# HuttleyLab/DiverseSeq

Hardware: AMD Instinct MI355X
Metric: sequences scored/sec (delta-JSD, k=6) (higher is better)
Workload: dtype f64 (results and every set update in f64; reject/accept decisions tiered: f32 and f32-log scores decide rows farther from the threshold than their proven error bands, f64 the rest)

## Files before the change

### diverseseq_amd/csrc/persist.hip

```cpp
#include "select_dev.h"

#include <algorithm>
#include <type_traits>
#include <cstddef>
#include <cstdlib>
#include <cstring>

namespace {

constexpr int P_THREADS = 512;
constexpr int P_J = 8;
constexpr int P_CH = 16;
constexpr uint32_t P_MAXN = 512;
constexpr uint32_t P_MAXN_BIG = 256;
constexpr uint32_t P_MAXN_MAX = 896;
constexpr uint32_t p_maxn(bool cached, bool maxm = false) { return cached ? (maxm ? P_MAXN_MAX : P_MAXN) : P_MAXN_BIG; }
constexpr uint32_t P_SMALLN = 16;
constexpr uint32_t P_SMALL_ROWS = 13;
constexpr uint32_t p_maxjobs(bool cached, bool maxm = false) { return p_maxn(cached, maxm) + 1; }
constexpr size_t p_acc_bytes(uint32_t maxn) { return size_t(8) * (maxn + 1) * 2 * sizeof(unsigned long long); }
__device__ __forceinline__ unsigned long long p_acc_word(double v) {
    return ((unsigned long long)__double2ll_rn(v * 0x1p50) << 6) + 1ull;
}
__device__ __forceinline__ double p_acc_value(unsigned long long w) { return double((long long)w >> 6) * 0x1p-50; }
// ... 2790 lines not shown
                        rec = __hip_atomic_load(&sync->wrec[epoch & 1u][q], RLX_AGENT);
                    if (p_word_listed(rec) != (l2 ? 1u : 0u)) wrong = true;
                    if (l2) {
                        unsigned long long ent = __hip_atomic_load(&sync->soft[epoch & 1u][q][0], RLX_AGENT);
                        for (uint32_t spins = 0; !p_word_is(ent, epoch) && spins < (1u << 20); spins++)
                            ent = __hip_atomic_load(&sync->soft[epoch & 1u][q][0], RLX_AGENT);
                        if (p_word_pos(ent, epoch) != uint64_t(epoch) * 4096u + 4001u + q) wrong = true;
                    }
                }
            }
            if (__ballot(wrong) != 0ull && lane == 0) fails++;
        }
        for (uint32_t z = (h >> 20) & 7u; z > 0; z--) __builtin_amdgcn_s_sleep(2);
        if (b < HO_MEMBERS * HO_K && tid < 8) {
            const double v = double((h >> 4) & 0xFFFFu) * (1.0 / 65536.0), v2 = double(h & 0xFFu) * (1.0 / 4096.0);
            p_acc_add(acc_all + (uint64_t(tid) * (HO_MEMBERS + 1) + b / HO_K) * 2, v, v2);
        }
        bool acc_ok = true, acc_wrong = false;
        if (tid < HO_MEMBERS) {
            const unsigned long long d0 = p_acc_complete(acc + uint64_t(tid) * 2, s_prev + tid * 2, HO_K, acc_ok);
            const unsigned long long d1 = p_acc_complete(acc + uint64_t(tid) * 2 + 1, s_prev + tid * 2 + 1, HO_K, acc_ok);
            unsigned long long e0 = 0ull, e1 = 0ull;
            for (uint32_t q = 0; q < HO_K; q++) {
                const uint32_t h2 = ho_hash(epoch, tid * HO_K + q);
                e0 += p_acc_word(double((h2 >> 4) & 0xFFFFu) * (1.0 / 65536.0));
                e1 += p_acc_word(double(h2 & 0xFFu) * (1.0 / 4096.0));
            }
            acc_wrong = !acc_ok || d0 != e0 || d1 != e1;
        }
        if (__syncthreads_or(acc_wrong ? 1 : 0) && tid == 0) fails++;
        if (mirror && epoch + 1 < rounds) {
            if (tid == 0) __hip_atomic_store(&sync->wrec[(epoch + 1) & 1u][b], p_word(epoch + 1, SEL_NONE, false), RLX_AGENT);
            early_rec = epoch + 1;
            for (uint32_t z = (h >> 16) & 15u; z > 0; z--) __builtin_amdgcn_s_sleep(16);
        }
    }
    if (tid == 0 && fails) atomicAdd(bad, fails);
    if (tid == 0 && __hip_atomic_load(&sync->timeout, RLX_AGENT)) atomicAdd(bad, 1ull << 32);
}

}

template <typename T>
static const void *persist_fn(const dvs_select *s) {
    const bool cached = s->dev.B <= uint64_t(P_J) * P_THREADS;
    if (s->params.mode == DVS_MODE_MAX) return reinterpret_cast<const void *>(persist_nmost_kernel<T, true, true>);
    if constexpr (std::is_same_v<T, uint16_t>) {
        if (s->persist_small) return reinterpret_cast<const void *>(persist_nmost_kernel<T, true, false, true>);
    }
    return cached ? reinterpret_cast<const void *>(persist_nmost_kernel<T, true>)
                  : reinterpret_cast<const void *>(persist_nmost_kernel<T, false>);
}

static int persist_prepare(dvs_ctx *ctx, dvs_select *s, uint32_t head_stop, hipStream_t on) {
    std::vector<unsigned char> &image = head_stop ? s->h_psync_head : s->h_psync;
    image.assign(sizeof(PSync), 0);
    PSync &init = *reinterpret_cast<PSync *>(image.data());
    init.stop_at = head_stop;
    init.seeded = s->persist_seeded ? 1u : 0u;
    init.seed_list = static_cast<const unsigned long long *>(s->d_seed_list);
    for (int g = 0; g < 8; g++) init.rel[g].hint = ~0ull;
    init.wg_thresh = s->params.window ? 0u : 4u;
    init.wg_scale = 1.5f;
    if (ctx->knobs.persist_wg_rounds >= 0) init.wg_thresh = uint32_t(ctx->knobs.persist_wg_rounds);
    init.no_coarse = (ctx->knobs.persist_no_coarse ? 1u : 0u) | (ctx->knobs.persist_no_events ? 2u : 0u) |
                     0u;
    init.small_rows = s->persist_small ? s->persist_small_rows : 0u;
    init.lds_bytes = uint32_t(s->persist_lds);
    init.wmax = uint32_t(std::min<uint64_t>(s->npos, 0xFFFFFFFFull));
    DVS_HIP(ctx, hipMemcpyAsync(head_stop ? s->psync_head : s->psync, &init, sizeof init, hipMemcpyHostToDevice, on));
    DVS_HIP(ctx, hipMemsetAsync(head_stop ? s->ppart_head : s->ppart, 0, p_acc_bytes(s->persist_maxn), on));
    return DVS_OK;
}

template <typename T>
static int persist_launch(dvs_ctx *ctx, dvs_select *s, const T *mat, uint32_t grid, uint32_t head_stop,
                          hipStream_t on) {
    const SelDev &d = s->dev;
    if (head_stop ? !s->head_prepared : !s->persist_prepared) {
        int prc = persist_prepare(ctx, s, head_stop, on);
        if (prc) return prc;
    }
    if (head_stop) s->head_prepared = false;
    else s->persist_prepared = false;
    s->persist_seeded = false;
    hipEvent_t e0 = nullptr, e1 = nullptr;
    if (s->time_scan) {
        if (s->ev_used + 2 > s->ev_pool.size()) {
            hipEvent_t a = dvs_event_get(ctx), b = dvs_event_get(ctx);
            s->ev_pool.push_back(a);
            s->ev_pool.push_back(b);
        }
        e0 = s->ev_pool[s->ev_used];
        e1 = s->ev_pool[s->ev_used + 1];
        s->ev_used += 2;
        (void)hipEventRecord(e0, on);
    }
    const void *fn = persist_fn<T>(s);
    SelDev d_arg = d;
    const T *mat_arg = mat;
    PSync *sync_arg = static_cast<PSync *>(head_stop ? s->psync_head : s->psync);
    unsigned long long *part_arg = static_cast<unsigned long long *>(head_stop ? s->ppart_head : s->ppart);
    uint32_t g_arg = grid;
    void *args[] = {&d_arg, &mat_arg, &sync_arg, &part_arg, &g_arg};
    hipError_t le = hipLaunchKernel(fn, dim3(grid), dim3(P_THREADS), args, s->persist_lds, on);
    if (s->time_scan) (void)hipEventRecord(e1, on);
    if (le != hipSuccess) {
        (void)hipGetLastError();
        return DVS_ERR_UNSUPPORTED;
    }
    DVS_HIP(ctx, hipGetLastError());
    return DVS_OK;
}

int dvs_persist_setup(dvs_ctx *ctx, dvs_select *s) {
    const uint64_t B = s->dev.B;
    s->persist = false;
    if (ctx->knobs.no_persist || ctx->persist_timeouts >= 3) return DVS_OK;
    if (ctx->knobs.cu_mask_set) return DVS_OK;
    const bool maxm = s->params.mode == DVS_MODE_MAX;
    if ((s->params.mode != DVS_MODE_NMOST && !maxm) || !s->h_order.empty() || !s->h_labels.empty()) return DVS_OK;
    if (s->npos >= P_POS_NONE) return DVS_OK;
    s->persist_grid = uint32_t(std::min(ctx->n_cu, int(P_MAXG)));
    const bool cached = B <= uint64_t(P_J) * P_THREADS;
    if (maxm && !cached) return DVS_OK;
// ... 31 lines not shown
        auto hit = ctx->persist_fits.find(key);
        if (hit == ctx->persist_fits.end()) {
            int per_cu = 0;
            const bool fits = hipOccupancyMaxActiveBlocksPerMultiprocessor(&per_cu, fn, P_THREADS, lds) == hipSuccess && per_cu >= 1;
            if (!fits) (void)hipGetLastError();
            hit = ctx->persist_fits.emplace(key, fits).first;
        }
        if (!hit->second) return DVS_OK;
    }
    rc = dvs_dev_alloc(ctx, &s->psync, sizeof(PSync), "persistent sync block");
    if (!rc) rc = dvs_dev_alloc(ctx, &s->ppart, p_acc_bytes(s->persist_maxn) + (maxm ? 2 * p_batch_bytes() : 0),
                                "leave-one-out accumulators");
    if (rc) return rc;
    s->persist = true;
    return DVS_OK;
}

size_t dvs_persist_dbg_offset(void) { return offsetof(PSync, dbg2); }
#ifdef DVS_PERSIST_STAMPS
size_t dvs_persist_trace_offset(void) { return offsetof(PSync, trace); }
#else
size_t dvs_persist_trace_offset(void) { return 0; }
#endif
#if defined(DVS_PERSIST_STAMPS) && defined(DVS_PROBE)
int dvs_persist_probe_id(void) { return DVS_PROBE; }
#else
int dvs_persist_probe_id(void) { return 0; }
#endif

int dvs_persist_launch(dvs_ctx *ctx, dvs_select *s) {
    return dvs_mat_dispatch(s->mat, [&](auto *mp) { return persist_launch(ctx, s, mp, s->persist_grid, 0u, ctx->stream); });
}

static int persist_head_blocks(dvs_ctx *ctx, dvs_select *s) {
    if (s->psync_head) return DVS_OK;
    int rc = dvs_dev_alloc(ctx, &s->psync_head, sizeof(PSync), "head phase sync block");
    if (!rc) rc = dvs_dev_alloc(ctx, &s->ppart_head, p_acc_bytes(s->persist_maxn), "head phase accumulators");
    return rc;
}

int dvs_persist_launch_head(dvs_ctx *ctx, dvs_select *s, uint32_t grid, uint32_t stop_at, hipStream_t on) {
    int rc = persist_head_blocks(ctx, s);
    if (rc) return rc;
    return dvs_mat_dispatch(s->mat, [&](auto *mp) { return persist_launch(ctx, s, mp, grid, stop_at, on); });
}

int dvs_persist_prepare_head(dvs_ctx *ctx, dvs_select *s, uint32_t stop_at, hipStream_t on) {
    int rc = persist_head_blocks(ctx, s);
    if (!rc) rc = persist_prepare(ctx, s, stop_at, on);
    if (!rc) s->head_prepared = true;
    return rc;
}

int dvs_persist_prepare_main(dvs_ctx *ctx, dvs_select *s) {
    int rc = persist_prepare(ctx, s, 0u, ctx->stream);
    if (!rc) s->persist_prepared = true;
    return rc;
}

extern "C" int dvs_selftest_handover(dvs_ctx *ctx, uint32_t rounds, uint64_t *failures) {
    if (!ctx || !failures || !rounds) return dvs_set_error(ctx, DVS_ERR_VALUE, "bad argument");
    if (rounds >= P_EPOCH_MAX) return dvs_set_error(ctx, DVS_ERR_VALUE, "at most %u rounds", P_EPOCH_MAX - 1);
    DVS_HIP(ctx, hipSetDevice(ctx->device));
    const uint32_t G = uint32_t(std::min(ctx->n_cu, int(P_MAXG)));
    if (G < HO_MEMBERS * HO_K + 2 || ctx->knobs.cu_mask_set)
        return dvs_set_error(ctx, DVS_ERR_UNSUPPORTED, "the self-test wants %u co-resident workgroups", HO_MEMBERS * HO_K + 2);
    void *d_sync = nullptr, *d_acc = nullptr, *d_bad = nullptr;
    int rc = dvs_dev_alloc(ctx, &d_sync, sizeof(PSync), "self-test sync block");
    if (!rc) rc = dvs_dev_alloc(ctx, &d_acc, p_acc_bytes(HO_MEMBERS), "self-test accumulators");
    if (!rc) rc = dvs_dev_alloc(ctx, &d_bad, 8, "self-test counter");
    if (!rc) {
        std::vector<unsigned char> image(sizeof(PSync), 0);
        PSync &init = *reinterpret_cast<PSync *>(image.data());
        for (int g = 0; g < 8; g++) init.rel[g].hint = ~0ull;
        hipError_t e = hipMemcpyAsync(d_sync, image.data(), sizeof(PSync), hipMemcpyHostToDevice, ctx->stream);
        if (e == hipSuccess) e = hipMemsetAsync(d_acc, 0, p_acc_bytes(HO_MEMBERS), ctx->stream);
        if (e == hipSuccess) e = hipMemsetAsync(d_bad, 0, 8, ctx->stream);
        if (e == hipSuccess) e = hipStreamSynchronize(ctx->stream);
        if (e == hipSuccess) {
            hipLaunchKernelGGL(handover_selftest_kernel, dim3(G), dim3(P_THREADS), 0, ctx->stream, static_cast<PSync *>(d_sync),
                               static_cast<unsigned long long *>(d_acc), G, rounds, static_cast<unsigned long long *>(d_bad));
            e = hipGetLastError();
        }
        unsigned long long bad = 0;
        if (e == hipSuccess) e = hipMemcpyAsync(&bad, d_bad, 8, hipMemcpyDeviceToHost, ctx->stream);
        if (e == hipSuccess) e = hipStreamSynchronize(ctx->stream);
        if (e != hipSuccess) rc = dvs_hip_fail(ctx, e, "hand-over self-test");
        *failures = bad;
    }
    dvs_dev_free(ctx, d_sync);
    dvs_dev_free(ctx, d_acc);
    dvs_dev_free(ctx, d_bad);
    return rc;
}
```

### diverseseq_amd/csrc/select.h

```cpp
#pragma once

#include "dvs_internal.h"

#define SEL_NONE 0xFFFFFFFFFFFFFFFFull
#define SEL_SEEDS_AT 512

enum : uint32_t { SEL_RUN = 0, SEL_DONE = 1, SEL_ARBITER = 2, SEL_ERROR = 3,
                  SEL_NEED_SETUP = 4 };
enum : uint32_t { ARB_RESOLVE = 1, ARB_FINALIZE = 2 };
enum : uint32_t { FORCE_NONE = 0, FORCE_ACCEPT = 1, FORCE_REJECT = 2, FORCE_COMMIT = 3, FORCE_ROLLBACK = 4 };

struct SelCtl {
    unsigned long long cursor;
    unsigned long long npos;
    unsigned long long event_pos;
    unsigned long long arb_pos;
    unsigned long long rows_scored, rows_rechecked;
    unsigned long long rows_coarse_passed;
    unsigned long long rows_before_launch;
    uint32_t window, window_min, window_max;
    uint32_t status, arb_stage, forced, forced_lowest;
    uint32_t size, lowest, mode, max_size, stat;
    uint32_t ev_kind;
    uint32_t ev_n;
// ... 18 lines not shown
    SelCtl *ctl = nullptr;
    uint64_t B = 0;
    uint32_t nlabels = 0;
    const uint32_t *order = nullptr;
    const uint32_t *labels = nullptr;
    const uint32_t *totals = nullptr;
    const double *rowH = nullptr;
    double *S = nullptr;
    double *Stmp = nullptr;
    double *base = nullptr;
    double *cand = nullptr;
    double *M = nullptr;
    double *mH = nullptr;
    double *mDelta = nullptr;
    double *dtmp = nullptr;
    double *dsum = nullptr;
    uint32_t *mLabel = nullptr;
    unsigned long long *mPos = nullptr;
    uint32_t *ord = nullptr;
    uint8_t *inset = nullptr;
    uint32_t *wg_rows = nullptr;
    unsigned long long *evlog_pos = nullptr;
    uint32_t *evlog_kind = nullptr;
    const double *gather_all = nullptr;
    uint32_t gather_world = 0;
    double *rowlog = nullptr;
    uint32_t rowlog_cap = 0;
};

struct dvs_select {
    dvs_ctx *ctx = nullptr;
    dvs_select_params params{};
    const dvs_matrix *mat = nullptr;
    int mat_kind = 0;
    uint64_t npos = 0;
    uint32_t cap = 0;
    SelDev dev;
    SelCtl *h_ctl = nullptr;
    SelCtl ctl0{};
    std::vector<uint32_t> h_order, h_labels;
    std::vector<uint32_t> h_out_labels;
    std::vector<uint64_t> seed_positions;
    uint32_t scan_grid = 0, loo_grid = 0;
    size_t scan_lds = 0;
    bool base_in_lds = true;
    bool scan_hot = false;
    bool persist = false;
    bool persist_fell_back = false;
    uint32_t persist_grid = 0, persist_maxn = 0, persist_maxjobs = 0;
    bool persist_small = false;
    uint32_t persist_small_rows = 0;
    size_t persist_lds = 0;
    void *psync = nullptr;
    std::vector<unsigned char> h_psync;
    std::vector<unsigned char> h_psync_head;
    void *ppart = nullptr;
    double *d_mbres = nullptr;
    uint32_t mb_jw = 0;
    uint32_t mb_launched = 0;
    void *psync_head = nullptr, *ppart_head = nullptr;
    bool persist_seeded = false;
    bool seeded_start = false;
    bool head_prepared = false;
    bool persist_prepared = false;
    bool used_side_streams = false;
    hipEvent_t ev_side_done = nullptr;
    void *d_seed_list = nullptr;
    bool seed_list_in_ctl = false;
    bool inset_clean = false;
    hipStream_t setup_side = nullptr;
    bool head_phase = false;
    int batch = 16;
    bool time_scan = false;
    std::vector<hipEvent_t> ev_pool;
    size_t ev_used = 0;
    double scan_ms = 0.0;
    double scan_ms_last = 0.0;
    uint64_t scan_launches = 0;
    uint32_t n_arbitrated = 0;
    double arbiter_ms = 0.0;
    bool fast_step = false;
    bool fs_need_scan = false;
    unsigned long long *h_fshist = nullptr;
    unsigned long long fs_launches = 0;
    unsigned long long fs_peek_floor = 0;
    double *fs_slot = nullptr;
    double *fs_packed = nullptr;
    double *d_jobres = nullptr;
    void *d_fsync = nullptr;
    uint32_t fs_K = 1, fs_jobs = 0, fs_grid = 0;
    size_t fs_lds = 0;
    std::vector<double> h_rowlog;
    uint64_t rowlog_have = 0;
    uint32_t steps_since_poll = 0;
    void *arbiter = nullptr;
};

int dvs_select_arbitrate(dvs_ctx *ctx, dvs_select *s);
void dvs_select_arbiter_free(dvs_select *s);

int dvs_persist_setup(dvs_ctx *ctx, dvs_select *s);
int dvs_persist_launch(dvs_ctx *ctx, dvs_select *s);
int dvs_persist_launch_head(dvs_ctx *ctx, dvs_select *s, uint32_t grid, uint32_t stop_at, hipStream_t on);
int dvs_persist_prepare_main(dvs_ctx *ctx, dvs_select *s);
int dvs_persist_prepare_head(dvs_ctx *ctx, dvs_select *s, uint32_t stop_at, hipStream_t on);
size_t dvs_persist_dbg_offset(void);
size_t dvs_persist_trace_offset(void);
int dvs_persist_probe_id(void);
```

### diverseseq_amd/csrc/select.hip

```cpp
#include "dvs_internal.h"
#include "select.h"
#include "select_dev.h"

#include <algorithm>
#include <chrono>
#include <type_traits>
#include <cmath>
#include <cstring>
#include <cstdlib>

namespace {

constexpr int SCAN_THREADS = 512;
constexpr int WIDE_THREADS = 1024;
constexpr int LOO_THREADS = 256;

template <typename T>
__device__ __forceinline__ void scan_rows_hot(SelCtl *ctl, const T *__restrict__ mat,
                                              const uint32_t *__restrict__ totals,
                                              const double *__restrict__ rowH, const double *bvec,
                                              uint64_t B, const ScanState &st, uint64_t first,
                                              uint64_t stride, uint32_t lane, uint32_t &nread,
                                              uint32_t &nprecise) {
    for (uint64_t r = first; r < st.nrows; r += stride) {
// ... 1693 lines not shown
}

__global__ __launch_bounds__(LOO_THREADS) void gather_members_kernel(SelDev d, double *__restrict__ rows,
                                                                    double *__restrict__ meta) {
    const uint32_t r = blockIdx.x, n = d.ctl->size;
    double *out = rows + uint64_t(r) * d.B;
    if (r >= n) {
        for (uint64_t i = threadIdx.x; i < d.B; i += LOO_THREADS) out[i] = 0.0;
        if (threadIdx.x == 0) meta[2 * r] = meta[2 * r + 1] = 0.0;
        return;
    }
    const uint32_t slot = d.ord[r];
    const double *src = d.M + uint64_t(slot) * d.B;
    for (uint64_t i = threadIdx.x; i < d.B; i += LOO_THREADS) out[i] = src[i];
    if (threadIdx.x == 0) {
        meta[2 * r] = double(d.mPos[slot]);
        meta[2 * r + 1] = 1.0;
    }
}

template <typename T>
__global__ __launch_bounds__(LOO_THREADS) void pack_event_kernel(SelDev d, const T *__restrict__ mat,
                                                                double *__restrict__ slot) {
    pack_event_body<T>(d, mat, slot);
}

}

static void sel_free(dvs_select *s) {
    if (!s) return;
#ifdef DVS_FS_TRACE
    if (s->d_jobres && getenv("DVS_FS_DEBUG")) {
        std::vector<unsigned long long> t(8 * 1024);
        (void)hipDeviceSynchronize();
        if (hipMemcpy(t.data(), reinterpret_cast<char *>(s->d_jobres) + size_t(2048) * 8 * 8, t.size() * 8, hipMemcpyDeviceToHost) == hipSuccess) {
            unsigned long long t0 = ~0ull;
            for (uint32_t b = 0; b < s->fs_grid; b++) if (t[b * 8]) t0 = std::min(t0, t[b * 8]);
            auto us = [&](unsigned long long x) { return x ? (double(x) - double(t0)) / 100.0 : -1.0; };
            double mx[8] = {0}, mn[8]; for (int k = 0; k < 8; k++) mn[k] = 1e9;
            for (uint32_t b = 1; b < s->fs_grid; b++) for (int k = 0; k < 7; k++) if (t[b * 8 + k]) { mx[k] = std::max(mx[k], us(t[b * 8 + k])); mn[k] = std::min(mn[k], us(t[b * 8 + k])); }
            fprintf(stderr, "[fs trace] scanning workgroups (us, min/max): start %.1f/%.1f decided %.1f/%.1f base+arrived %.1f/%.1f scan end %.1f/%.1f\n", mn[0], mx[0], mn[1], mx[1], mn[2], mx[2], mn[6], mx[6]);
            std::vector<double> e, r1, c1, sc; double posted = -1; unsigned long long nr = 0, nrmax = 0;
            for (uint32_t b = 1; b < s->fs_grid; b++) { if (t[b * 8 + 6]) e.push_back(us(t[b * 8 + 6])); if (t[b * 8 + 3]) r1.push_back(us(t[b * 8 + 3])); if (t[b * 8 + 4]) c1.push_back(us(t[b * 8 + 4]));
                if (t[b * 8 + 5]) sc.push_back(us(t[b * 8 + 5])); nr += t[b * 8 + 7]; nrmax = std::max(nrmax, t[b * 8 + 7]); }
            std::sort(e.begin(), e.end()); std::sort(r1.begin(), r1.end()); std::sort(c1.begin(), c1.end()); std::sort(sc.begin(), sc.end());
            auto pc = [&](std::vector<double> &v, double q) { return v.empty() ? -1.0 : v[size_t(q * (v.size() - 1))]; };
            fprintf(stderr, "[fs trace] wave 0s: scan loop entered p10/50/90/max %.1f %.1f %.1f %.1f; first row's data there %.1f %.1f %.1f %.1f; its score %.1f %.1f %.1f %.1f; scan end %.1f %.1f %.1f %.1f; first post (wave 0s only) %.1f; rows read sum %llu max %llu\n",
                    pc(sc, .1), pc(sc, .5), pc(sc, .9), pc(sc, 1), pc(r1, .1), pc(r1, .5), pc(r1, .9), pc(r1, 1), pc(c1, .1), pc(c1, .5), pc(c1, .9), pc(c1, 1), pc(e, .1), pc(e, .5), pc(e, .9), pc(e, 1), posted, nr, nrmax);
            const uint32_t L = 0;
            fprintf(stderr, "[fs trace] state writer: start %.1f decided %.1f loaded %.1f all arrived %.1f small stores issued %.1f rows issued %.1f done %.1f\n", us(t[L * 8]), us(t[L * 8 + 1]), us(t[L * 8 + 2]), us(t[L * 8 + 3]), us(t[L * 8 + 4]), us(t[L * 8 + 6]), us(t[L * 8 + 5]));
        }
    }
#endif
    if (s->used_side_streams && s->ctx) {
        if (s->ctx->stream_head) (void)hipStreamSynchronize(s->ctx->stream_head);
        if (s->ctx->stream2) (void)hipStreamSynchronize(s->ctx->stream2);
    }
    void *ptrs[] = {s->dev.ctl, s->dev.S, s->dev.Stmp, s->dev.base, s->dev.cand, s->dev.M,
                    s->dev.mH, s->dev.mDelta, s->dev.dtmp, s->dev.dsum, s->dev.mLabel, s->dev.mPos,
                    s->dev.ord, s->dev.inset, s->dev.wg_rows, s->dev.evlog_pos, s->dev.evlog_kind, s->dev.rowlog,
                    (void *)s->dev.order, (void *)s->dev.labels};
    for (void *p : ptrs)
        dvs_dev_free(s->ctx, p);
    if (s->h_fshist && s->fs_launches && s->ctx) (void)hipStreamSynchronize(s->ctx->stream);
    dvs_pinned_put(s->ctx, s->h_ctl);
    if (s->h_fshist) dvs_pinned_put(s->ctx, s->h_fshist);
    for (hipEvent_t e : s->ev_pool) dvs_event_put(s->ctx, e);
    dvs_dev_free(s->ctx, s->d_mbres);
    dvs_dev_free(s->ctx, s->d_jobres);
    dvs_dev_free(s->ctx, s->d_fsync);
    dvs_dev_free(s->ctx, s->psync);
    dvs_dev_free(s->ctx, s->ppart);
    dvs_dev_free(s->ctx, s->psync_head);
    dvs_dev_free(s->ctx, s->ppart_head);
    if (!s->seed_list_in_ctl) dvs_dev_free(s->ctx, s->d_seed_list);
    if (s->ev_side_done) dvs_event_put(s->ctx, s->ev_side_done);
    dvs_select_arbiter_free(s);
    dvs_ctx_release(s->ctx);
    delete s;
}

template <typename T>
static void launch_iteration(dvs_ctx *ctx, dvs_select *s, const T *mat, int stage, hipStream_t on = nullptr) {
    const SelDev &d = s->dev;
    const hipStream_t stream = on ? on : ctx->stream;
    if (stage == 0) {
        hipEvent_t e0 = nullptr, e1 = nullptr;
        if (s->time_scan) {
            if (s->ev_used + 2 > s->ev_pool.size()) {
                hipEvent_t a = dvs_event_get(ctx), b = dvs_event_get(ctx);
                s->ev_pool.push_back(a);
                s->ev_pool.push_back(b);
            }
            e0 = s->ev_pool[s->ev_used];
            e1 = s->ev_pool[s->ev_used + 1];
            s->ev_used += 2;
            (void)hipEventRecord(e0, stream);
        }
        if (s->scan_hot)
            hipLaunchKernelGGL((scan_kernel<T, true>), dim3(s->scan_grid), dim3(SCAN_THREADS),
                               s->scan_lds, stream, d.ctl, mat, d.totals, d.rowH, d.order, d.labels,
                               d.inset, d.nlabels, d.base, d.wg_rows, d.B, s->base_in_lds ? 1 : 0);
        else
            hipLaunchKernelGGL((scan_kernel<T, false>), dim3(s->scan_grid), dim3(SCAN_THREADS),
                               s->scan_lds, stream, d.ctl, mat, d.totals, d.rowH, d.order, d.labels,
                               d.inset, d.nlabels, d.base, d.wg_rows, d.B, s->base_in_lds ? 1 : 0);
        if (s->time_scan) (void)hipEventRecord(e1, stream);
    }
    if (stage <= 1)
        hipLaunchKernelGGL((resolve_kernel<T>), dim3(1), dim3(WIDE_THREADS), 0, stream, d, mat);
    hipLaunchKernelGGL(loo_kernel, dim3(s->loo_grid + 1), dim3(LOO_THREADS), 0, stream, d, s->scan_grid);
    hipLaunchKernelGGL(finalize_kernel, dim3(1), dim3(WIDE_THREADS), 0, stream, d);
}

template <typename T>
static int launch_max_batch(dvs_ctx *ctx, dvs_select *s, const T *mat, uint32_t size_bound) {
    if (!s->d_mbres) {
        s->mb_jw = std::min<uint32_t>(s->cap, MB_MAX_MEMBERS) + 3;
        int rc = dvs_dev_alloc(ctx, (void **)&s->d_mbres, size_t(3) * MB_ROWS * s->mb_jw * sizeof(double), "max batch results");
        if (rc) return rc;
    }
    if (size_bound + 3 > s->mb_jw) return DVS_OK;
    hipLaunchKernelGGL((max_batch_jobs_kernel<T>), dim3(size_bound + 3, MB_ROWS / MB_RG), dim3(MB_THREADS), 0, ctx->stream, s->dev, mat,
                       s->d_mbres, s->mb_jw);
    hipLaunchKernelGGL(max_batch_decide_kernel, dim3(1), dim3(WIDE_THREADS), 0, ctx->stream, s->dev, s->d_mbres, s->mb_jw);
    s->mb_launched++;
    return DVS_OK;
}

static int sel_poll(dvs_ctx *ctx, dvs_select *s) {
    DVS_HIP(ctx, hipMemcpyAsync(s->h_ctl, s->dev.ctl, sizeof(SelCtl), hipMemcpyDeviceToHost,
                                ctx->stream));
    DVS_HIP(ctx, hipStreamSynchronize(ctx->stream));
    return DVS_OK;
}

template <typename T>
static int sel_seed(dvs_ctx *ctx, dvs_select *s, const T *mat, hipStream_t st, bool light = false);

template <typename T>
static int sel_run_loop(dvs_ctx *ctx, dvs_select *s, const T *mat, bool first_unpolled = false) {
    unsigned long long persist_cursor = 0;
    unsigned persist_launches = 0;
    bool persist_was_last = false;
    unsigned persist_idle = 0;
    bool mb_seen = false, mb_dense = true;
    unsigned long long mb_cursor = 0, mb_events = 0;
    bool mb_useful = true;
    uint32_t mb_rows_seen = 0, mb_round_pairs = 0, mb_idle_rounds = 0;
    if (s->persist && first_unpolled) {
        persist_cursor = s->params.n_seed;
        persist_launches = 1;
        persist_was_last = true;
        int rc0 = dvs_persist_launch(ctx, s);
        if (rc0 == DVS_ERR_UNSUPPORTED) {
            s->persist = false;
            s->persist_fell_back = true;
            persist_launches = 0;
            if (s->seeded_start) {
                s->seeded_start = false;
                s->persist_seeded = false;
                int src = sel_seed<T>(ctx, s, mat, ctx->stream);
                if (src) return src;
            }
        } else if (rc0) {
            return rc0;
        }
    }
    for (;;) {
        int rc = sel_poll(ctx, s);
        if (rc) return rc;
        const SelCtl &c = *s->h_ctl;
        if (s->time_scan && s->ev_used) {
            for (size_t i = 0; i + 1 < s->ev_used; i += 2) {
                float ms = 0.f;
                if (hipEventElapsedTime(&ms, s->ev_pool[i], s->ev_pool[i + 1]) == hipSuccess) {
                    s->scan_ms += ms;
                    s->scan_ms_last = ms;
                }
                s->scan_launches++;
            }
            s->ev_used = 0;
        }
        for (int which = 0; which < 2 && s->persist && ctx->knobs.persist_debug; which++) {
            unsigned long long dbg[32];
            void *blk = which ? s->psync : s->psync_head;
            if (!blk) continue;
            if (hipMemcpy(dbg, static_cast<char *>(blk) + dvs_persist_dbg_offset(), sizeof dbg, hipMemcpyDeviceToHost) == hipSuccess) {
                fprintf(stderr, "[dvs persist] %s launch\n", which ? "full-grid" : "head-phase");
                if (dvs_persist_probe_id()) {
                    fprintf(stderr, "[dvs persist probe %d] block 0 (owns a job): %.3f us x %llu; the last scanning block (no job): %.3f us x %llu\n",
// ... 157 lines not shown
                    return rc;
                } else {
                    continue;
                }
            }
        }
        if (replica_full) persist_was_last = false;
        const int iters = (s->persist && !replica_full && persist_launches && !persist_was_last && persist_idle < 2) ? 1 : s->batch;
        if (mb_seen) {
            const unsigned long long rows = c.cursor - mb_cursor, evs = c.n_events - mb_events;
            if (rows) mb_dense = evs * 2 >= rows;
        }
        mb_seen = true;
        mb_cursor = c.cursor;
        mb_events = c.n_events;
        if (mb_round_pairs) mb_useful = (c.mb_rows - mb_rows_seen) >= 2u * mb_round_pairs;
        mb_rows_seen = c.mb_rows;
        mb_round_pairs = 0;
        const bool mb_can = mb_dense && iters > 1 && c.mode == DVS_MODE_MAX && c.size < c.max_size && c.s_is_resum != 0 &&
                            !(s->params.flags & DVS_SELECT_STEPWISE);
        const bool mb_probe = mb_can && !mb_useful && ++mb_idle_rounds >= 4;
        if (mb_probe || mb_useful) mb_idle_rounds = 0;
        const int mb_iters = !mb_can ? 0 : mb_useful ? iters : mb_probe ? 2 : 0;
        for (int i = 0; i < iters; i++) {
            for (int b = 0; i < mb_iters && b < 3; b++) {
                if ((rc = launch_max_batch<T>(ctx, s, mat, c.size + uint32_t(i)))) return rc;
                mb_round_pairs += b == 0;
            }
            launch_iteration<T>(ctx, s, mat, 0);
        }
        DVS_HIP(ctx, hipGetLastError());
    }
}

static void sel_plan_setup_stream(dvs_ctx *ctx, dvs_select *s) {
    s->setup_side = nullptr;
    s->head_phase = false;
    if (s->mat->head_rows_built && s->params.n_seed <= s->mat->head_rows_built && s->h_order.empty() &&
        !(s->params.flags & DVS_SELECT_STEPWISE)) {
        s->head_phase = s->mat->rest_beside_head && ctx->stream_head && s->persist &&
                        s->params.mode == DVS_MODE_NMOST && s->params.window == 0 &&
                        s->cap + 2 <= uint32_t(ctx->head_cus) && s->npos > 4ull * s->mat->head_rows_built &&
                        s->params.n_seed + 64 <= s->mat->head_rows_built && !ctx->knobs.no_head_phase;
        s->setup_side = s->head_phase ? ctx->stream_head : dvs_ctx_stream2(ctx);
    }
}

template <typename T>
static int sel_start(dvs_ctx *ctx, dvs_select *s, const T *mat) {
    hipStream_t side = s->setup_side;
    const bool head_phase = s->head_phase;
    hipStream_t st = side ? side : ctx->stream;
    if (side) s->used_side_streams = true;
    int rc = sel_seed<T>(ctx, s, mat, st, s->seeded_start);
    if (rc) return rc;
    if (head_phase) {
        rc = dvs_persist_launch_head(ctx, s, uint32_t(ctx->head_cus), s->mat->head_rows_built, side);
        if (rc && rc != DVS_ERR_UNSUPPORTED) return rc;
        if (rc == DVS_ERR_UNSUPPORTED && s->seeded_start) {
            s->seeded_start = false;
            s->persist_seeded = false;
            rc = sel_seed<T>(ctx, s, mat, st);
            if (rc) return rc;
        }
        rc = dvs_persist_prepare_main(ctx, s);
        if (rc) return rc;
        const_cast<dvs_matrix *>(s->mat)->rest_beside_head = false;
    }
    if (side) {
        if (!s->ev_side_done) s->ev_side_done = dvs_event_get(ctx);
        DVS_HIP(ctx, hipEventRecord(s->ev_side_done, side));
        DVS_HIP(ctx, hipStreamWaitEvent(ctx->stream, s->ev_side_done, 0));
    }
    if (s->params.flags & DVS_SELECT_STEPWISE) return sel_poll(ctx, s);
    return sel_run_loop<T>(ctx, s, mat, true);
}

template <typename T>
static int sel_seed(dvs_ctx *ctx, dvs_select *s, const T *mat, hipStream_t st, bool light) {
    const std::vector<uint64_t> &seeds = s->seed_positions;
    SelDev &d = s->dev;
    SelCtl c = s->ctl0;
    const uint32_t wdef = s->params.window ? s->params.window : (s->persist ? s->persist_grid * 2u : 4096u);
    c.window_min = wdef;
    c.window_max = std::max<uint32_t>(wdef, s->scan_grid * (SCAN_THREADS / 64) * 8);
    c.window = wdef;
    *s->h_ctl = c;
    if (!s->inset_clean || st != (s->setup_side ? s->setup_side : ctx->stream))
        DVS_HIP(ctx, hipMemsetAsync(d.inset, 0, std::max<size_t>(d.nlabels, 1), st));
    s->inset_clean = false;
    if (!s->d_seed_list) {
        int rc0 = dvs_dev_alloc(ctx, &s->d_seed_list, seeds.size() * sizeof(uint64_t), "seed list");
        if (rc0) return rc0;
    }
    uint64_t *d_seed = static_cast<uint64_t *>(s->d_seed_list);
    if (s->seed_list_in_ctl) {
        std::memcpy(reinterpret_cast<unsigned char *>(s->h_ctl) + SEL_SEEDS_AT, seeds.data(), seeds.size() * sizeof(uint64_t));
        DVS_HIP(ctx, hipMemcpyAsync(d.ctl, s->h_ctl, SEL_SEEDS_AT + seeds.size() * sizeof(uint64_t), hipMemcpyHostToDevice, st));
    } else {
        DVS_HIP(ctx, hipMemcpyAsync(d.ctl, s->h_ctl, sizeof c, hipMemcpyHostToDevice, st));
        DVS_HIP(ctx, hipMemcpyAsync(d_seed, seeds.data(), seeds.size() * sizeof(uint64_t),
                                    hipMemcpyHostToDevice, st));
    }
    if (light) {
        DVS_HIP(ctx, hipGetLastError());
        return DVS_OK;
    }
    hipLaunchKernelGGL((seed_kernel<T>), dim3(uint32_t(seeds.size())), dim3(LOO_THREADS), 0,
                       st, s->dev, mat, d_seed);
    hipLaunchKernelGGL(rebuild_sum_kernel, dim3(uint32_t((s->dev.B + RSUM_THREADS - 1) / RSUM_THREADS)), dim3(RSUM_THREADS), 0, st, s->dev);
    hipLaunchKernelGGL(rebuild_kernel, dim3(1), dim3(WIDE_THREADS), 0, st, s->dev);
    launch_iteration<T>(ctx, s, mat, 2, st);
    DVS_HIP(ctx, hipGetLastError());
    return DVS_OK;
}

extern "C" int dvs_select_run(dvs_ctx *ctx, const dvs_matrix *m, const uint32_t *order,
                              const uint32_t *labels, uint64_t npos,
                              const dvs_select_params *params, dvs_select **out) {
    if (!ctx || !m || !params || !out) return dvs_set_error(ctx, DVS_ERR_VALUE, "null argument");
    *out = nullptr;
    DVS_HIP(ctx, hipSetDevice(ctx->device));
    const uint64_t B = m->nbins;
    if (!order && npos > m->nrows)
        return dvs_set_error(ctx, DVS_ERR_VALUE, "npos %llu exceeds the matrix rows %u",
                             (unsigned long long)npos, m->nrows);
    uint32_t n_seed = params->n_seed;
    uint32_t max_size = params->max_size;
    if (params->mode == DVS_MODE_SET) n_seed = uint32_t(npos);
    const uint32_t *caller_labels = nullptr;
    if (labels && !order && params->mode != DVS_MODE_SET) {
        bool distinct = true;
        bool rising = true;
        for (uint64_t p = 1; p < npos && rising; p++) rising = labels[p] > labels[p - 1];
        if (!rising) {
            std::vector<uint32_t> sorted(labels, labels + npos);
            std::sort(sorted.begin(), sorted.end());
            for (uint64_t p = 1; p < npos && distinct; p++)
                distinct = sorted[p] != sorted[p - 1] || sorted[p] == 0xFFFFFFFFu;
        }
        if (distinct) {
            caller_labels = labels;
            labels = nullptr;
        }
    }
    if (npos < n_seed)
        return dvs_set_error(ctx, DVS_ERR_VALUE, "The number of sequences %llu is < n %u",
                             (unsigned long long)npos, n_seed);
    if (params->mode == DVS_MODE_MAX && npos <= max_size) max_size = uint32_t(npos);
    if (params->mode != DVS_MODE_MAX) max_size = n_seed;

    uint32_t nlabels = 0;
    if (order || labels) {
        for (uint64_t p = 0; p < npos; p++) {
            const uint32_t row = order ? order[p] : uint32_t(p);
            if (row == DVS_ROW_REMOTE) continue;
// ... 101 lines not shown
        d.rowlog_cap = uint32_t(ring);
        SEL_ALLOC(d.rowlog, size_t(ring) * B * 8);
        uint32_t fsK = 1;
        while (uint64_t(cap + 1) * fsK * 2 <= 96 && uint64_t(fsK) * 2 * FS_JOB_THREADS <= B) fsK *= 2;
        const size_t fs_lds = ((B + 1) & ~1ull) * 16 + size_t(cap + 1) * 3 * 8 + size_t(cap + 1) * fsK * 7 * 8 + 64;
        if (params->mode == DVS_MODE_NMOST && params->n_seed >= 2 && !labels && !ctx->knobs.no_fast_step && fs_lds <= ctx->lds_per_block &&
            uint64_t(cap + 1) <= FS_MAXJOBS) {
            s->fs_K = fsK;
            s->fs_lds = fs_lds;
            s->fs_grid = uint32_t(ctx->n_cu);
            SEL_ALLOC(s->d_jobres, size_t(FS_MAXJOBS) * FS_RES * 8 + 8 * 8 * 1024);
            SEL_HIP(hipMemsetAsync(s->d_jobres, 0, size_t(FS_MAXJOBS) * FS_RES * 8 + 8 * 8 * 1024, ctx->stream));
            SEL_ALLOC(s->d_fsync, sizeof(FsSync));
            SEL_HIP(hipMemsetAsync(s->d_fsync, 0, sizeof(FsSync), ctx->stream));
            void *hh = nullptr;
            if (dvs_pinned_get(ctx, &hh) == DVS_OK) {
                memset(hh, 0, 4096);
                s->h_fshist = static_cast<unsigned long long *>(hh);
            }
            s->fast_step = true;
            s->fs_need_scan = true;
        }
    }
    if (order) {
        SEL_ALLOC(d.order, size_t(npos) * 4);
        SEL_HIP(hipMemcpyAsync((void *)d.order, order, size_t(npos) * 4, hipMemcpyHostToDevice,
                                    ctx->stream));
    }
    if (labels) {
        SEL_ALLOC(d.labels, size_t(npos) * 4);
        SEL_HIP(hipMemcpyAsync((void *)d.labels, labels, size_t(npos) * 4,
                                    hipMemcpyHostToDevice, ctx->stream));
    }
#undef SEL_ALLOC

    static_assert(sizeof(SelCtl) <= 4096, "control block must fit a cached pinned block");
    {
        int prc = dvs_pinned_get(ctx, (void **)&s->h_ctl);
        if (prc) {
            sel_free(s);
            return prc;
        }
    }

    {
        int prc = dvs_persist_setup(ctx, s);
        if (prc) {
            sel_free(s);
            return prc;
        }
    }
    sel_plan_setup_stream(ctx, s);
    if (s->setup_side) s->used_side_streams = true;
    SEL_HIP(hipMemsetAsync(d.inset, 0, std::max<size_t>(nlabels, 1), s->setup_side ? s->setup_side : ctx->stream));
    s->inset_clean = true;
    SEL_HIP(hipMemsetAsync(d.wg_rows, 0, size_t(s->scan_grid) * 8, s->setup_side ? s->setup_side : ctx->stream));
    s->seeded_start = s->persist && params->mode == DVS_MODE_NMOST && B <= 4096 && !order && !labels &&
                      !(s->params.flags & DVS_SELECT_STEPWISE) && n_seed >= 2 && n_seed <= 32 && !ctx->knobs.persist_no_seeded;
    s->persist_seeded = s->seeded_start;
    if (size_t(n_seed) * sizeof(uint64_t) <= 4096 - SEL_SEEDS_AT) {
        s->d_seed_list = reinterpret_cast<unsigned char *>(d.ctl) + SEL_SEEDS_AT;
        s->seed_list_in_ctl = true;
    } else if (s->seeded_start) {
        int arc = dvs_dev_alloc(ctx, &s->d_seed_list, size_t(n_seed) * sizeof(uint64_t), "seed list");
        if (arc) {
            sel_free(s);
            return arc;
        }
    }
    if (s->persist && m->rest_beside_head && ctx->stream_head && m->head_rows_built && params->mode == DVS_MODE_NMOST &&
        !order && !labels) {
        s->used_side_streams = true;
        int prc = dvs_persist_prepare_head(ctx, s, m->head_rows_built, ctx->stream_head);
        if (prc) {
            sel_free(s);
            return prc;
        }
    }
    std::vector<uint64_t> seeds;
    {
        std::vector<uint32_t> h_tot(n_seed);
        {
            int src = dvs_matrix_settle(ctx, m);
            if (src) {
                sel_free(s);
                return src;
            }
        }
        hipError_t ce = hipSuccess;
        if (!order && n_seed && n_seed <= m->h_head_totals.size()) {
            std::copy(m->h_head_totals.begin(), m->h_head_totals.begin() + n_seed, h_tot.begin());
        } else if (!order && n_seed) {
            ce = hipMemcpyAsync(h_tot.data(), m->d_totals, size_t(n_seed) * 4, hipMemcpyDeviceToHost, ctx->stream);
        } else {
            for (uint64_t p = 0; p < n_seed && ce == hipSuccess; p++)
                ce = hipMemcpyAsync(&h_tot[p], m->d_totals + order[p], 4, hipMemcpyDeviceToHost, ctx->stream);
        }
        if ((order || n_seed > m->h_head_totals.size()) &&
            (hipStreamSynchronize(ctx->stream) != hipSuccess || ce != hipSuccess)) {
            sel_free(s);
            return dvs_set_error(ctx, DVS_ERR_RUNTIME, "reading the seed rows' totals failed");
        }
        for (uint64_t p = 0; p < n_seed; p++)
            if (h_tot[p] > 0) seeds.push_back(p);
    }
    if (seeds.size() < 2) {
        sel_free(s);
        return seeds.empty() ? dvs_set_error(ctx, DVS_ERR_VALUE, "records cannot be empty")
                             : dvs_set_error(ctx, DVS_ERR_VALUE, "must have > 1 KmerSeq");
    }

    SelCtl c;
    std::memset(&c, 0, sizeof c);
    c.cursor = n_seed;
    c.npos = npos;
    c.event_pos = SEL_NONE;
    c.status = SEL_RUN;
    c.size = uint32_t(seeds.size());
    c.mode = params->mode;
    c.max_size = max_size;
    c.stat = params->stat;
    c.forced = FORCE_NONE;
    c.forced_lowest = 0xFFFFFFFFu;
    c.band = 0.0;
// ... 452 lines not shown
```

Baseline: 69.63 million.

## Fuse persistent-kernel setup copies and memsets into one device init kernel

Replaces the host-built sync-block image, its host-to-device copy and the accumulator memset with a small device kernel that zeroes and fills the sync headers itself. On the seeded head-phase path, one launch also initialises both sync blocks, the inset flags, the per-workgroup row counters and the control block with its seed list, replacing several separate async copies and memsets. The aim is to cut per-call launch and API overhead on short runs. It also skips the redundant side-stream synchronisation at free time once the side stream has been joined and drained, at the cost of more state flags to keep consistent.

```diff
diff --git a/diverseseq_amd/csrc/persist.hip b/diverseseq_amd/csrc/persist.hip
--- a/diverseseq_amd/csrc/persist.hip
+++ b/diverseseq_amd/csrc/persist.hip
@@ -2866,25 +2866,96 @@
                   : reinterpret_cast<const void *>(persist_nmost_kernel<T, false>);
 }
 
+constexpr size_t P_HDR_BYTES = offsetof(PSync, wrec);
+static_assert(P_HDR_BYTES % 8 == 0 && sizeof(PSync) % 8 == 0, "the sync block is set up in 8-byte words");
+constexpr uint32_t P_CTL_WORDS = (SEL_SEEDS_AT + 32 * 8) / 8;
+
+struct PInitSync {
+    PSync *sync;
+    unsigned long long *part;
+    uint32_t part_words;
+    uint32_t stop_at, seeded, wg_thresh, no_coarse, small_rows, lds_bytes, wmax;
+    float wg_scale;
+    const unsigned long long *seed_list;
+};
+struct PInitArgs {
+    PInitSync one[2];
+    uint32_t n_sync;
+    uint32_t inset_bytes, wg_words, ctl_words;
+    unsigned char *inset;
+    unsigned long long *wg_rows;
+    unsigned long long *ctl;
+    unsigned long long ctl_img[P_CTL_WORDS];
+};
+constexpr int P_INIT_THREADS = 256;
+constexpr uint32_t P_INIT_GRID = 32;
+
+__global__ __launch_bounds__(P_INIT_THREADS) void persist_init_kernel(const PInitArgs a) {
+    __shared__ unsigned long long img[P_HDR_BYTES / 8];
+    const uint32_t tid = threadIdx.x;
+    if (blockIdx.x < a.n_sync) {
+        const PInitSync &o = a.one[blockIdx.x];
+        for (uint32_t i = tid; i < P_HDR_BYTES / 8; i += P_INIT_THREADS) img[i] = 0ull;
+        __syncthreads();
+        if (tid == 0) {
+            PSync &h = *reinterpret_cast<PSync *>(img);
+            h.wg_thresh = o.wg_thresh;
+            h.wg_scale = o.wg_scale;
+            h.no_coarse = o.no_coarse;
+            h.stop_at = o.stop_at;
+            h.seeded = o.seeded;
+            h.seed_list = o.seed_list;
+            h.small_rows = o.small_rows;
+            h.lds_bytes = o.lds_bytes;
+            h.wmax = o.wmax;
+            for (int g = 0; g < 8; g++) h.rel[g].hint = ~0ull;
+        }
+        __syncthreads();
+        unsigned long long *dst = reinterpret_cast<unsigned long long *>(o.sync);
+        for (uint32_t i = tid; i < P_HDR_BYTES / 8; i += P_INIT_THREADS) dst[i] = img[i];
+    }
+    constexpr uint32_t body = uint32_t((sizeof(PSync) - P_HDR_BYTES) / 8);
+    const uint32_t stride = gridDim.x * P_INIT_THREADS;
+    const uint32_t i0 = blockIdx.x * P_INIT_THREADS + tid;
+    for (uint32_t q = 0; q < a.n_sync; q++) {
+        unsigned long long *dst = reinterpret_cast<unsigned long long *>(a.one[q].sync) + P_HDR_BYTES / 8;
+        for (uint32_t i = i0; i < body; i += stride) dst[i] = 0ull;
+        for (uint32_t i = i0; i < a.one[q].part_words; i += stride) a.one[q].part[i] = 0ull;
+    }
+    for (uint32_t i = i0; i < a.wg_words; i += stride) a.wg_rows[i] = 0ull;
+    for (uint32_t i = i0; i < a.ctl_words; i += stride) a.ctl[i] = a.ctl_img[i];
+    for (uint32_t i = i0; i < a.inset_bytes; i += stride) a.inset[i] = 0;
+}
+
+static PInitSync persist_init_sync(dvs_ctx *ctx, const dvs_select *s, uint32_t head_stop) {
+    PInitSync o{};
+    o.sync = static_cast<PSync *>(head_stop ? s->psync_head : s->psync);
+    o.part = static_cast<unsigned long long *>(head_stop ? s->ppart_head : s->ppart);
+    o.part_words = uint32_t(p_acc_bytes(s->persist_maxn) / 8);
+    o.stop_at = head_stop;
+    o.seeded = s->persist_seeded ? 1u : 0u;
+    o.seed_list = static_cast<const unsigned long long *>(s->d_seed_list);
+    o.wg_thresh = s->params.window ? 0u : 4u;
+    o.wg_scale = 1.5f;
+    if (ctx->knobs.persist_wg_rounds >= 0) o.wg_thresh = uint32_t(ctx->knobs.persist_wg_rounds);
+    o.no_coarse = (ctx->knobs.persist_no_coarse ? 1u : 0u) | (ctx->knobs.persist_no_events ? 2u : 0u);
+    o.small_rows = s->persist_small ? s->persist_small_rows : 0u;
+    o.lds_bytes = uint32_t(s->persist_lds);
+    o.wmax = uint32_t(std::min<uint64_t>(s->npos, 0xFFFFFFFFull));
+    return o;
+}
+
+static int persist_init_launch(dvs_ctx *ctx, const PInitArgs &a, hipStream_t on) {
+    hipLaunchKernelGGL(persist_init_kernel, dim3(P_INIT_GRID), dim3(P_INIT_THREADS), 0, on, a);
+    DVS_HIP(ctx, hipGetLastError());
+    return DVS_OK;
+}
+
 static int persist_prepare(dvs_ctx *ctx, dvs_select *s, uint32_t head_stop, hipStream_t on) {
-    std::vector<unsigned char> &image = head_stop ? s->h_psync_head : s->h_psync;
-    image.assign(sizeof(PSync), 0);
-    PSync &init = *reinterpret_cast<PSync *>(image.data());
-    init.stop_at = head_stop;
-    init.seeded = s->persist_seeded ? 1u : 0u;
-    init.seed_list = static_cast<const unsigned long long *>(s->d_seed_list);
-    for (int g = 0; g < 8; g++) init.rel[g].hint = ~0ull;
-    init.wg_thresh = s->params.window ? 0u : 4u;
-    init.wg_scale = 1.5f;
-    if (ctx->knobs.persist_wg_rounds >= 0) init.wg_thresh = uint32_t(ctx->knobs.persist_wg_rounds);
-    init.no_coarse = (ctx->knobs.persist_no_coarse ? 1u : 0u) | (ctx->knobs.persist_no_events ? 2u : 0u) |
-                     0u;
-    init.small_rows = s->persist_small ? s->persist_small_rows : 0u;
-    init.lds_bytes = uint32_t(s->persist_lds);
-    init.wmax = uint32_t(std::min<uint64_t>(s->npos, 0xFFFFFFFFull));
-    DVS_HIP(ctx, hipMemcpyAsync(head_stop ? s->psync_head : s->psync, &init, sizeof init, hipMemcpyHostToDevice, on));
-    DVS_HIP(ctx, hipMemsetAsync(head_stop ? s->ppart_head : s->ppart, 0, p_acc_bytes(s->persist_maxn), on));
-    return DVS_OK;
+    PInitArgs a{};
+    a.one[0] = persist_init_sync(ctx, s, head_stop);
+    a.n_sync = 1;
+    return persist_init_launch(ctx, a, on);
 }
 
 template <typename T>
@@ -3022,6 +3093,31 @@
     return rc;
 }
 
+int dvs_persist_init_head(dvs_ctx *ctx, dvs_select *s, uint32_t stop_at, hipStream_t on, size_t ctl_bytes) {
+    if (ctl_bytes > size_t(P_CTL_WORDS) * 8 || (ctl_bytes & 7u) || !s->persist_seeded)
+        return dvs_set_error(ctx, DVS_ERR_RUNTIME, "head-phase set-up: %zu bytes of control block", ctl_bytes);
+    int rc = persist_head_blocks(ctx, s);
+    if (rc) return rc;
+    PInitArgs a{};
+    a.one[0] = persist_init_sync(ctx, s, stop_at);
+    s->persist_seeded = false;
+    a.one[1] = persist_init_sync(ctx, s, 0u);
+    s->persist_seeded = true;
+    a.n_sync = 2;
+    a.inset = s->dev.inset;
+    a.inset_bytes = uint32_t(std::max<size_t>(s->dev.nlabels, 1));
+    a.wg_rows = reinterpret_cast<unsigned long long *>(s->dev.wg_rows);
+    a.wg_words = s->scan_grid;
+    a.ctl = reinterpret_cast<unsigned long long *>(s->dev.ctl);
+    a.ctl_words = uint32_t(ctl_bytes / 8);
+    std::memcpy(a.ctl_img, s->h_ctl, ctl_bytes);
+    rc = persist_init_launch(ctx, a, on);
+    if (rc) return rc;
+    s->head_prepared = true;
+    s->persist_prepared = true;
+    return DVS_OK;
+}
+
 int dvs_persist_prepare_main(dvs_ctx *ctx, dvs_select *s) {
     int rc = persist_prepare(ctx, s, 0u, ctx->stream);
     if (!rc) s->persist_prepared = true;
diff --git a/diverseseq_amd/csrc/select.h b/diverseseq_amd/csrc/select.h
--- a/diverseseq_amd/csrc/select.h
+++ b/diverseseq_amd/csrc/select.h
@@ -94,8 +94,6 @@
     uint32_t persist_small_rows = 0;
     size_t persist_lds = 0;
     void *psync = nullptr;
-    std::vector<unsigned char> h_psync;
-    std::vector<unsigned char> h_psync_head;
     void *ppart = nullptr;
     double *d_mbres = nullptr;
     uint32_t mb_jw = 0;
@@ -106,6 +104,9 @@
     bool head_prepared = false;
     bool persist_prepared = false;
     bool used_side_streams = false;
+    bool init_fused = false;
+    bool side_joined = false;
+    bool side_drained = false;
     hipEvent_t ev_side_done = nullptr;
     void *d_seed_list = nullptr;
     bool seed_list_in_ctl = false;
@@ -146,6 +147,7 @@
 int dvs_persist_launch_head(dvs_ctx *ctx, dvs_select *s, uint32_t grid, uint32_t stop_at, hipStream_t on);
 int dvs_persist_prepare_main(dvs_ctx *ctx, dvs_select *s);
 int dvs_persist_prepare_head(dvs_ctx *ctx, dvs_select *s, uint32_t stop_at, hipStream_t on);
+int dvs_persist_init_head(dvs_ctx *ctx, dvs_select *s, uint32_t stop_at, hipStream_t on, size_t ctl_bytes);
 size_t dvs_persist_dbg_offset(void);
 size_t dvs_persist_trace_offset(void);
 int dvs_persist_probe_id(void);
diff --git a/diverseseq_amd/csrc/select.hip b/diverseseq_amd/csrc/select.hip
--- a/diverseseq_amd/csrc/select.hip
+++ b/diverseseq_amd/csrc/select.hip
@@ -1769,7 +1769,7 @@
         }
     }
 #endif
-    if (s->used_side_streams && s->ctx) {
+    if (s->used_side_streams && s->ctx && !s->side_drained) {
         if (s->ctx->stream_head) (void)hipStreamSynchronize(s->ctx->stream_head);
         if (s->ctx->stream2) (void)hipStreamSynchronize(s->ctx->stream2);
     }
@@ -1849,11 +1849,13 @@
     DVS_HIP(ctx, hipMemcpyAsync(s->h_ctl, s->dev.ctl, sizeof(SelCtl), hipMemcpyDeviceToHost,
                                 ctx->stream));
     DVS_HIP(ctx, hipStreamSynchronize(ctx->stream));
+    if (s->side_joined) s->side_drained = true;
     return DVS_OK;
 }
 
 template <typename T>
 static int sel_seed(dvs_ctx *ctx, dvs_select *s, const T *mat, hipStream_t st, bool light = false);
+static size_t sel_ctl_image(dvs_select *s);
 
 template <typename T>
 static int sel_run_loop(dvs_ctx *ctx, dvs_select *s, const T *mat, bool first_unpolled = false) {
@@ -2117,7 +2119,13 @@
     const bool head_phase = s->head_phase;
     hipStream_t st = side ? side : ctx->stream;
     if (side) s->used_side_streams = true;
-    int rc = sel_seed<T>(ctx, s, mat, st, s->seeded_start);
+    int rc;
+    if (s->init_fused) {
+        rc = dvs_persist_init_head(ctx, s, s->mat->head_rows_built, side, sel_ctl_image(s));
+        s->inset_clean = true;
+    } else {
+        rc = sel_seed<T>(ctx, s, mat, st, s->seeded_start);
+    }
     if (rc) return rc;
     if (head_phase) {
         rc = dvs_persist_launch_head(ctx, s, uint32_t(ctx->head_cus), s->mat->head_rows_built, side);
@@ -2128,7 +2136,7 @@
             rc = sel_seed<T>(ctx, s, mat, st);
             if (rc) return rc;
         }
-        rc = dvs_persist_prepare_main(ctx, s);
+        if (!s->init_fused) rc = dvs_persist_prepare_main(ctx, s);
         if (rc) return rc;
         const_cast<dvs_matrix *>(s->mat)->rest_beside_head = false;
     }
@@ -2137,20 +2145,29 @@
         DVS_HIP(ctx, hipEventRecord(s->ev_side_done, side));
         DVS_HIP(ctx, hipStreamWaitEvent(ctx->stream, s->ev_side_done, 0));
     }
+    s->side_joined = side && s->init_fused;
     if (s->params.flags & DVS_SELECT_STEPWISE) return sel_poll(ctx, s);
     return sel_run_loop<T>(ctx, s, mat, true);
 }
 
-template <typename T>
-static int sel_seed(dvs_ctx *ctx, dvs_select *s, const T *mat, hipStream_t st, bool light) {
+static size_t sel_ctl_image(dvs_select *s) {
     const std::vector<uint64_t> &seeds = s->seed_positions;
-    SelDev &d = s->dev;
     SelCtl c = s->ctl0;
     const uint32_t wdef = s->params.window ? s->params.window : (s->persist ? s->persist_grid * 2u : 4096u);
     c.window_min = wdef;
     c.window_max = std::max<uint32_t>(wdef, s->scan_grid * (SCAN_THREADS / 64) * 8);
     c.window = wdef;
     *s->h_ctl = c;
+    if (!s->seed_list_in_ctl) return sizeof c;
+    std::memcpy(reinterpret_cast<unsigned char *>(s->h_ctl) + SEL_SEEDS_AT, seeds.data(), seeds.size() * sizeof(uint64_t));
+    return SEL_SEEDS_AT + seeds.size() * sizeof(uint64_t);
+}
+
+template <typename T>
+static int sel_seed(dvs_ctx *ctx, dvs_select *s, const T *mat, hipStream_t st, bool light) {
+    const std::vector<uint64_t> &seeds = s->seed_positions;
+    SelDev &d = s->dev;
+    const size_t ctl_bytes = sel_ctl_image(s);
     if (!s->inset_clean || st != (s->setup_side ? s->setup_side : ctx->stream))
         DVS_HIP(ctx, hipMemsetAsync(d.inset, 0, std::max<size_t>(d.nlabels, 1), st));
     s->inset_clean = false;
@@ -2159,14 +2176,10 @@
         if (rc0) return rc0;
     }
     uint64_t *d_seed = static_cast<uint64_t *>(s->d_seed_list);
-    if (s->seed_list_in_ctl) {
-        std::memcpy(reinterpret_cast<unsigned char *>(s->h_ctl) + SEL_SEEDS_AT, seeds.data(), seeds.size() * sizeof(uint64_t));
-        DVS_HIP(ctx, hipMemcpyAsync(d.ctl, s->h_ctl, SEL_SEEDS_AT + seeds.size() * sizeof(uint64_t), hipMemcpyHostToDevice, st));
-    } else {
-        DVS_HIP(ctx, hipMemcpyAsync(d.ctl, s->h_ctl, sizeof c, hipMemcpyHostToDevice, st));
+    DVS_HIP(ctx, hipMemcpyAsync(d.ctl, s->h_ctl, ctl_bytes, hipMemcpyHostToDevice, st));
+    if (!s->seed_list_in_ctl)
         DVS_HIP(ctx, hipMemcpyAsync(d_seed, seeds.data(), seeds.size() * sizeof(uint64_t),
                                     hipMemcpyHostToDevice, st));
-    }
     if (light) {
         DVS_HIP(ctx, hipGetLastError());
         return DVS_OK;
@@ -2374,9 +2387,6 @@
     }
     sel_plan_setup_stream(ctx, s);
     if (s->setup_side) s->used_side_streams = true;
-    SEL_HIP(hipMemsetAsync(d.inset, 0, std::max<size_t>(nlabels, 1), s->setup_side ? s->setup_side : ctx->stream));
-    s->inset_clean = true;
-    SEL_HIP(hipMemsetAsync(d.wg_rows, 0, size_t(s->scan_grid) * 8, s->setup_side ? s->setup_side : ctx->stream));
     s->seeded_start = s->persist && params->mode == DVS_MODE_NMOST && B <= 4096 && !order && !labels &&
                       !(s->params.flags & DVS_SELECT_STEPWISE) && n_seed >= 2 && n_seed <= 32 && !ctx->knobs.persist_no_seeded;
     s->persist_seeded = s->seeded_start;
@@ -2390,8 +2400,14 @@
             return arc;
         }
     }
-    if (s->persist && m->rest_beside_head && ctx->stream_head && m->head_rows_built && params->mode == DVS_MODE_NMOST &&
-        !order && !labels) {
+    s->init_fused = s->head_phase && s->seeded_start && s->seed_list_in_ctl;
+    if (!s->init_fused) {
+        SEL_HIP(hipMemsetAsync(d.inset, 0, std::max<size_t>(nlabels, 1), s->setup_side ? s->setup_side : ctx->stream));
+        s->inset_clean = true;
+        SEL_HIP(hipMemsetAsync(d.wg_rows, 0, size_t(s->scan_grid) * 8, s->setup_side ? s->setup_side : ctx->stream));
+    }
+    if (!s->init_fused && s->persist && m->rest_beside_head && ctx->stream_head && m->head_rows_built &&
+        params->mode == DVS_MODE_NMOST && !order && !labels) {
         s->used_side_streams = true;
         int prc = dvs_persist_prepare_head(ctx, s, m->head_rows_built, ctx->stream_head);
         if (prc) {
```

New measurement: 71.66 million (median of 6 runs). 2.9% higher.
